# microsoft/foldingdiff

Measured on AMD Instinct MI355X. Metric: backbones/sec (L=128, T=1000, bs=512), higher is better.
Workload: dtype f32 (fp16 hi/lo split operands, 3x v_mfma_f32_{32x32x16,16x16x32}_f16 per product, fp32 accumulate)

## Files before the change

### foldingdiff_amd/csrc/ffn16.hip

```cpp
#include <cstdlib>
#include <type_traits>

#include "fdmi_kernels.h"
#include "img_common.h"
#include "launch_common.h"

namespace fdmi {
namespace ffn {

typedef float f32x4 __attribute__((ext_vector_type(4)));
typedef const __attribute__((address_space(3))) u32x4* lds_cu128_t;
__device__ __forceinline__ unsigned lds_addr(const void* p) { return (unsigned)(unsigned long long)(lds_ptr_t)(const_cast<void*>(p)); }
__device__ __forceinline__ u32x4 lds_u128(unsigned a) { return *(lds_cu128_t)(unsigned long long)a; }
__device__ __forceinline__ f16x8 lds_f16x8(unsigned a) { return __builtin_bit_cast(f16x8, lds_u128(a)); }

__device__ __forceinline__ void swap16(unsigned& vdst, unsigned& src) {
  const auto r = __builtin_amdgcn_permlane16_swap(vdst, src, false, false);
  vdst = r[0];
  src = r[1];
}
__device__ __forceinline__ float quad_sum(float x) {
  unsigned a = __builtin_bit_cast(unsigned, x), b = a;
  swap32(a, b);
  float m = __builtin_bit_cast(float, a) + __builtin_bit_cast(float, b);
  a = __builtin_bit_cast(unsigned, m);
  b = a;
  swap16(a, b);
  return __builtin_bit_cast(float, a) + __builtin_bit_cast(float, b);
}

template <int V> using IC = std::integral_constant<int, V>;
template <int LO, int HI, class F>
__device__ __forceinline__ void static_for(F&& f) {
  if constexpr (LO < HI) {
    f(IC<LO>{});
    static_for<LO + 1, HI>(f);
  }
}

#ifndef FDMI_FFN_DBG
#define FDMI_FFN_DBG 0
#endif
#ifndef FDMI_FFN_ST_AUX
#define FDMI_FFN_ST_AUX 0
#endif
#ifndef FDMI_FFN_PRIO
#define FDMI_FFN_PRIO 2
#endif

__device__ __forceinline__ f32x4 mfma16(const f16x8& a, const f16x8& b, const f32x4& c) {
  return __builtin_amdgcn_mfma_f32_16x16x32_f16(a, b, c, 0, 0, 0);
}

constexpr int NW = 8;
constexpr int TILE = 2048;
constexpr int STEP = 4 * TILE;
constexpr int SPS = 2;
constexpr int STAGE = SPS * STEP;
constexpr int NST = 3;
constexpr int PPW = STAGE / 1024 / NW;
constexpr int OFF_W = 0;
constexpr int OFF_X = NST * STAGE;
__host__ __device__ constexpr int off_p(int nkt) { return OFF_X + NW * nkt * 1024; }

template <int NKT, bool TAIL, bool PROF>
__global__ __launch_bounds__(64 * NW) void ffn16_kernel(FfnArgs p) {
  static_assert(NKT == 12 || NKT == 6, "d_model 384 or 192, intermediate size 2 d_model");
  constexpr int D = 32 * NKT;
  constexpr int NG = NKT;
  constexpr int SPG = 2 * NKT;
  constexpr int STG = SPG / SPS;
  static_assert(STG % NST == 0, "a group is a whole number of ring turns: its first stage always sits in slot 0");
  constexpr int NSA = TAIL ? NKT * NKT / 2 : 0;
  static_assert((NSA / SPS) % NST == 0 && NSA % SPS == 0, "whole ring turns");
  constexpr int W_BYTES = (NSA / SPS + NG * STG) * STAGE;
  constexpr int OFF_P = off_p(NKT);
  constexpr int OFF_P1 = OFF_P + 5 * D * 4;
  extern __shared__ __attribute__((aligned(16))) unsigned char smem[];
  const int tid = threadIdx.x, lane = tid & 63;
  const int wq = __builtin_amdgcn_readfirstlane(tid >> 6);
  const int grp = wq >> 2;
  unsigned smem0 = __builtin_amdgcn_readfirstlane(lds_addr(smem));
  asm volatile("" : "+s"(smem0));
  auto lane_id = [&]() __attribute__((always_inline)) {
    int ln;
    asm volatile("v_mbcnt_lo_u32_b32 %0, -1, 0\n\tv_mbcnt_hi_u32_b32 %0, -1, %0" : "=v"(ln));
    return ln;
  };
  auto lane_off_of = [](int ln) __attribute__((always_inline)) { return (unsigned)((ln >> 4) * 256 + (ln & 15) * 16); };

  {
    float* par = reinterpret_cast<float*>(smem + OFF_P);
    for (int i = tid; i < 2 * D; i += 64 * NW) par[i] = p.bi[i];
    for (int i = tid; i < D; i += 64 * NW) {
      par[2 * D + i] = p.bd[i];
      par[3 * D + i] = p.gamma[i];
      par[4 * D + i] = p.beta[i] * p.out_scale;
      if constexpr (TAIL) {
        par[5 * D + i] = p.bo[i] * (1.0f / p.ao_scale);
        par[6 * D + i] = p.g1[i];
        par[7 * D + i] = p.b1[i] * p.a_scale;
      }
    }
  }

  int w_src = 0, w_slot = 0;
  const __amdgpu_buffer_rsrc_t rs_w = __builtin_amdgcn_make_buffer_rsrc(const_cast<unsigned char*>(p.wimg), 0, W_BYTES, 0x00020000);
  auto issue_w = [&]() __attribute__((always_inline)) {
    const lds_ptr_t dst = (lds_ptr_t)(unsigned long long)(smem0 + OFF_W + (unsigned)__builtin_amdgcn_readfirstlane(w_slot));
    const int so = __builtin_amdgcn_readfirstlane(w_src);
    const int vo = lane_id() * 16;
#pragma unroll
    for (int k = 0; k < PPW; ++k) dma16(rs_w, dst + (wq + NW * k) * 1024, vo, so + (wq + NW * k) * 1024);
    w_src = w_src + STAGE == W_BYTES ? 0 : w_src + STAGE;
    w_slot = w_slot + STAGE == NST * STAGE ? 0 : w_slot + STAGE;
  };

  f16x8 ah[NKT];
  const __amdgpu_buffer_rsrc_t rs_a =
      __builtin_amdgcn_make_buffer_rsrc(const_cast<unsigned char*>(TAIL ? p.cimg : p.aimg), 0, p.a_bytes, 0x00020000);
  const __amdgpu_buffer_rsrc_t rs_h = __builtin_amdgcn_make_buffer_rsrc(const_cast<unsigned char*>(TAIL ? p.hres : p.aimg), 0, p.a_bytes, 0x00020000);
  auto row_off = [&](int r0) __attribute__((always_inline)) {
    const int ln = lane_id();
    const int row = r0 + 16 * wq + (ln & 15);
    return (unsigned)(((row >> 5) * (NKT * 256) + (row & 31)) * 16 + (ln >> 4) * 512);
  };
  u32x4 tl[NKT];
  auto load_hi = [&](int r0) __attribute__((always_inline)) {
    const unsigned hoff = row_off(r0);
#pragma unroll
    for (int kt = 0; kt < NKT; ++kt)
      ah[kt] = __builtin_bit_cast(f16x8, __builtin_amdgcn_raw_buffer_load_b128(rs_a, (int)hoff, kt * 8 * 512, 0));
  };
  auto load_lo = [&](auto KT, unsigned hoff) __attribute__((always_inline)) {
    constexpr int kt = decltype(KT)::value;
    tl[kt] = __builtin_bit_cast(u32x4, __builtin_amdgcn_raw_buffer_load_b128(rs_a, (int)hoff, (kt * 8 + 4) * 512, 0));
  };
  auto commit_lo = [&]() __attribute__((always_inline)) {
    const unsigned ax = smem0 + OFF_X + (unsigned)(wq * NKT * 1024 + lane_id() * 16);
#pragma unroll
    for (int kt = 0; kt < NKT; ++kt) *(__attribute__((address_space(3))) u32x4*)(unsigned long long)(ax + (unsigned)(kt * 1024)) = tl[kt];
  };
  const __amdgpu_buffer_rsrc_t rs_o = __builtin_amdgcn_make_buffer_rsrc(p.out, 0, p.out_bytes, 0x00020000);
  auto load_res = [&](auto KT, unsigned hoff, f32x4 (&Yr)[2 * NKT]) __attribute__((always_inline)) {
    constexpr int kt = decltype(KT)::value;
    Yr[2 * kt] = __builtin_bit_cast(f32x4, __builtin_amdgcn_raw_buffer_load_b128(rs_h, (int)hoff, kt * 8 * 512, 0));
    Yr[2 * kt + 1] = __builtin_bit_cast(f32x4, __builtin_amdgcn_raw_buffer_load_b128(rs_h, (int)hoff, (kt * 8 + 4) * 512, 0));
  };

  const bool rec = PROF && blockIdx.x == 0 && p.stamps != nullptr;
  unsigned long long* stp = PROF ? p.stamps + (size_t)wq * 16 * 16 : nullptr;
  int slot = 0;
#define FD_STAMP(i) do { if (PROF) { if (rec && slot < 16 && lane == 0) stp[slot * 16 + (i)] = __builtin_amdgcn_s_memtime(); } } while (0)
#define FD_SB() __builtin_amdgcn_sched_barrier(0)
#define FD_STAMP_G(i) do { if (PROF) { if (rec && slot == 0 && G == 1 && lane == 0) stp[15 * 16 + (i)] = __builtin_amdgcn_s_memtime(); } } while (0)

  const int n_pass = p.dims ? min(p.panels, __builtin_amdgcn_readfirstlane(p.dims[1]) >> 7) : p.panels;
  if ((int)blockIdx.x >= n_pass) return;
  const float os_up = p.up_scale, os_dn = p.down_scale, hs = 0.5f * p.g_scale;
  const f32x4 zero4 = {0.f, 0.f, 0.f, 0.f};
  f32x4 Y[2 * NKT];
  f32x4 U[4];
  f32x4 Up[4];
  u32x4 uh[2], ul[2];

  load_hi((int)blockIdx.x * 128);
  {
    const unsigned hoff = row_off((int)blockIdx.x * 128);
    static_for<0, NKT>([&](auto KT) __attribute__((always_inline)) { load_lo(KT, hoff); });
    if constexpr (TAIL) static_for<0, NKT>([&](auto KT) __attribute__((always_inline)) { load_res(KT, hoff, Y); });
  }
  issue_w();
  issue_w();
  issue_w();
  FD_WAIT_VM(3 * PPW);
  commit_lo();
  FD_WAIT_VM(2 * PPW);
  barrier_keep_vm();

  auto gelu_piece = [&](auto P, unsigned abq) __attribute__((always_inline)) {
    constexpr int pc = decltype(P)::value, pr = pc >> 2, j = pc & 3;
    const u32x2 b = *(const __attribute__((address_space(3))) u32x2*)(unsigned long long)(abq + (unsigned)((32 * pr + 2 * j) * 4));
    float o0 = __builtin_fmaf(Up[2 * pr + (j >> 1)][2 * (j & 1)], os_up, __builtin_bit_cast(float, (unsigned)b[0]));
    float o1 = __builtin_fmaf(Up[2 * pr + (j >> 1)][2 * (j & 1) + 1], os_up, __builtin_bit_cast(float, (unsigned)b[1]));
#if !(FDMI_FFN_DBG & 1)
    const float h0 = o0 * hs, h1 = o1 * hs;
    o0 = __builtin_fmaf(h0, erf_rational(o0 * 0.70710678118654752440f), h0);
    o1 = __builtin_fmaf(h1, erf_rational(o1 * 0.70710678118654752440f), h1);
#endif
    unsigned a, c;
    split_pair(o0, o1, a, c);
    uh[pr][j] = a;
    ul[pr][j] = c;
  };

  auto steps = [&](auto S0, auto S1, auto GEL, unsigned abq) __attribute__((always_inline)) {
    constexpr int s0 = decltype(S0)::value, s1 = decltype(S1)::value;
    constexpr bool gel = decltype(GEL)::value == 1, pha = decltype(GEL)::value == 2;
    auto stage_top = [&]() __attribute__((always_inline)) {
      FD_WAIT_VM(PPW);
      barrier_keep_vm();
      issue_w();
    };
    f16x8 fx[4], fy[4], xl;
    unsigned a_W, a_X;
    {
      const int ln = lane_id();
      a_W = smem0 + OFF_W + lane_off_of(ln);
      a_X = smem0 + OFF_X + (unsigned)(wq * NKT * 1024 + ln * 16);
      asm volatile("" : "+v"(a_W), "+v"(a_X));
    }
    auto plane_reads = [&](auto S, auto LO, f16x8 (&f)[4]) __attribute__((always_inline)) {
      constexpr int s = decltype(S)::value, lo = decltype(LO)::value;
      constexpr unsigned off = (unsigned)(((s / SPS) % NST) * STAGE + (s % SPS) * STEP + lo * 1024);
#if FDMI_FFN_DBG & 8
      if constexpr (lo == 1) {
#pragma unroll
        for (int t = 0; t < 4; ++t) f[t] = fx[t];
      } else
#endif
#pragma unroll
      for (int t = 0; t < 4; ++t) f[t] = lds_f16x8(a_W + off + (unsigned)(t * TILE));
      if constexpr (pha) {
        if constexpr (lo == 0 && s % (NKT / 2) == 0) xl = lds_f16x8(a_X + (unsigned)((s / (NKT / 2)) * 1024));
      } else {
        if constexpr (lo == 0 && s < NKT) xl = lds_f16x8(a_X + (unsigned)(s * 1024));
      }
    };
    auto mm = [&](auto S, auto WHICH, const f16x8 (&f)[4]) __attribute__((always_inline)) {
      constexpr int s = decltype(S)::value, which = decltype(WHICH)::value;
      if constexpr (pha) {
        constexpr int kt = s / (NKT / 2), q = s % (NKT / 2);
#pragma unroll
        for (int t = 0; t < 4; ++t) Y[4 * q + t] = mfma16(f[t], which == 1 ? xl : ah[kt], Y[4 * q + t]);
      } else if constexpr (s < NKT) {
#if !(FDMI_FFN_DBG & 4)
#pragma unroll
        for (int t = 0; t < 4; ++t) U[t] = mfma16(f[t], which == 1 ? xl : ah[s], U[t]);
#endif
      } else {
#if !(FDMI_FFN_DBG & 2)
        constexpr int pr = (s - NKT) / (NKT / 2), q = (s - NKT) % (NKT / 2);
#pragma unroll
        for (int t = 0; t < 4; ++t) Y[4 * q + t] = mfma16(f[t], __builtin_bit_cast(f16x8, which == 1 ? ul[pr] : uh[pr]), Y[4 * q + t]);
#endif
      }
    };
    plane_reads(S0, IC<0>{}, fx);
    FD_SB();
    static_for<s0, s1>([&](auto S) __attribute__((always_inline)) {
      constexpr int s = decltype(S)::value;
      constexpr bool top = s % SPS == SPS - 1;
      plane_reads(S, IC<1>{}, fy);
      FD_SB();
      if constexpr (top) {
        if (grp == 0) stage_top();
      }
#if FDMI_FFN_PRIO
      __builtin_amdgcn_s_setprio(FDMI_FFN_PRIO);
#endif
      mm(S, IC<0>{}, fx);
      mm(S, IC<1>{}, fx);
#if FDMI_FFN_PRIO
      __builtin_amdgcn_s_setprio(0);
#endif
      FD_SB();
      if constexpr (top) {
        if (grp != 0) stage_top();
      }
      if constexpr (s + 1 < s1) plane_reads(IC<s + 1>{}, IC<0>{}, fx);
      FD_SB();
      if constexpr (gel) {
        if (grp == 0) {
          static_for<0, 8>([&](auto P) __attribute__((always_inline)) {
            if constexpr (1 + decltype(P)::value * (NKT - 2) / 8 == s) gelu_piece(P, abq);
          });
        }
        FD_SB();
      }
      mm(S, IC<2>{}, fy);
      FD_SB();
      if constexpr (gel) {
        if (grp != 0) {
          static_for<0, 8>([&](auto P) __attribute__((always_inline)) {
            if constexpr (1 + decltype(P)::value * (NKT - 2) / 8 == s) gelu_piece(P, abq);
          });
        }
        FD_SB();
      }
    });
  };

  for (int panel = blockIdx.x; panel < n_pass; panel += (int)gridDim.x) {
    FD_STAMP(0);
    if constexpr (TAIL) {
      const int ln = lane_id();
      const int g = ln >> 4;
      const unsigned pb1 = smem0 + OFF_P1 + (unsigned)(8 * g * 4);
      const unsigned ax = smem0 + OFF_X + (unsigned)(wq * NKT * 1024 + ln * 16);
      {
        const float c = p.hres_inv * (1.0f / p.ao_scale);
#pragma unroll
        for (int kt = 0; kt < NKT; ++kt) {
          const u32x4 rh = __builtin_bit_cast(u32x4, Y[2 * kt]), rl = __builtin_bit_cast(u32x4, Y[2 * kt + 1]);
          const u32x4 b0 = lds_u128(pb1 + (unsigned)(kt * 128)), b1 = lds_u128(pb1 + (unsigned)(kt * 128 + 16));
#pragma unroll
          for (int j = 0; j < 2; ++j)
#pragma unroll
            for (int e = 0; e < 4; e += 2) {
              const unsigned hw = rh[2 * j + e / 2], lw = rl[2 * j + e / 2];
              const unsigned bw0 = j == 0 ? b0[e] : b1[e], bw1 = j == 0 ? b0[e + 1] : b1[e + 1];
              float v0 = fma_mix_lo(hw, c, __builtin_bit_cast(float, bw0));
              float v1 = fma_mix_hi(hw, c, __builtin_bit_cast(float, bw1));
              Y[2 * kt + j][e] = fma_mix_lo(lw, c, v0);
              Y[2 * kt + j][e + 1] = fma_mix_hi(lw, c, v1);
            }
        }
      }
      steps(IC<0>{}, IC<NSA>{}, IC<2>{}, 0u);
      const float os_ao = p.ao_scale;
      float sum = 0.f;
#pragma unroll
      for (int t = 0; t < 2 * NKT; ++t)
#pragma unroll
        for (int e = 0; e < 4; ++e) {
          Y[t][e] *= os_ao;
          sum += Y[t][e];
        }
      const float inv_n = 1.0f / (float)D;
      float mean = quad_sum(sum) * inv_n;
      asm volatile("" : "+v"(mean));
      float t2 = 0.f;
#pragma unroll
      for (int t = 0; t < 2 * NKT; ++t)
#pragma unroll
        for (int e = 0; e < 4; ++e) {
          const float dl = Y[t][e] - mean;
          Y[t][e] = dl;
          t2 = __builtin_fmaf(dl, dl, t2);
        }
      const float rstd = (1.0f / sqrtf(__builtin_fmaf(quad_sum(t2), inv_n, p.eps1))) * p.a_scale;
#pragma unroll
      for (int kt = 0; kt < NKT; ++kt) {
        const u32x4 g0 = lds_u128(pb1 + (unsigned)(D * 4 + kt * 128)), g1 = lds_u128(pb1 + (unsigned)(D * 4 + kt * 128 + 16));
        const u32x4 e0 = lds_u128(pb1 + (unsigned)(2 * D * 4 + kt * 128)), e1 = lds_u128(pb1 + (unsigned)(2 * D * 4 + kt * 128 + 16));
        float o[8];
#pragma unroll
        for (int e = 0; e < 4; ++e) {
          o[e] = __builtin_fmaf(Y[2 * kt][e] * rstd, __builtin_bit_cast(float, (unsigned)g0[e]), __builtin_bit_cast(float, (unsigned)e0[e]));
          o[4 + e] = __builtin_fmaf(Y[2 * kt + 1][e] * rstd, __builtin_bit_cast(float, (unsigned)g1[e]), __builtin_bit_cast(float, (unsigned)e1[e]));
        }
        u32x4 hv, lv;
#pragma unroll
        for (int j = 0; j < 4; ++j) {
          unsigned a, b;
          split_pair(o[2 * j], o[2 * j + 1], a, b);
          hv[j] = a;
          lv[j] = b;
        }
        ah[kt] = __builtin_bit_cast(f16x8, hv);
        *(__attribute__((address_space(3))) u32x4*)(unsigned long long)(ax + (unsigned)(kt * 1024)) = lv;
      }
    }
#pragma unroll
    for (int t = 0; t < 2 * NKT; ++t) Y[t] = zero4;
#pragma unroll
    for (int t = 0; t < 4; ++t) U[t] = zero4;
    steps(IC<0>{}, IC<NKT>{}, IC<0>{}, 0u);
    for (int G = 0; G < NG; ++G) {
#pragma unroll
      for (int t = 0; t < 4; ++t) {
        Up[t] = U[t];
        U[t] = zero4;
      }
      unsigned abq = smem0 + OFF_P + (unsigned)((64 * G + 8 * (lane_id() >> 4)) * 4);
      asm volatile("" : "+v"(abq));
      FD_STAMP_G(0);
      FD_STAMP_G(1);
      if (G + 1 < NG) {
#ifdef FDMI_FFN_NOPIPE
        static_for<0, 8>([&](auto P) __attribute__((always_inline)) { gelu_piece(P, abq); });
        steps(IC<0>{}, IC<NKT>{}, IC<0>{}, abq);
#else
        steps(IC<0>{}, IC<NKT>{}, IC<1>{}, abq);
#endif
      } else {
        static_for<0, 8>([&](auto P) __attribute__((always_inline)) { gelu_piece(P, abq); });
      }
      FD_STAMP_G(2);
      steps(IC<NKT>{}, IC<SPG>{}, IC<0>{}, 0u);
      FD_STAMP_G(3);
      if (slot == 0) FD_STAMP(1 + (G < 12 ? G : 11));
    }
    {
      const int ln = lane_id();
      const int g = ln >> 4;
      const unsigned pb = smem0 + OFF_P + (unsigned)((2 * D + 8 * g) * 4);
      const unsigned ax = smem0 + OFF_X + (unsigned)(wq * NKT * 1024 + ln * 16);
      const float ri = p.resid_inv;
      float sum = 0.f;
#pragma unroll
      for (int kt = 0; kt < NKT; ++kt) {
        const u32x4 b0 = lds_u128(pb + (unsigned)(kt * 128)), b1 = lds_u128(pb + (unsigned)(kt * 128 + 16));
        const u32x4 rh = __builtin_bit_cast(u32x4, ah[kt]), rl = lds_u128(ax + (unsigned)(kt * 1024));
#pragma unroll
        for (int j = 0; j < 2; ++j)
#pragma unroll
          for (int e = 0; e < 4; e += 2) {
            const unsigned bw0 = j == 0 ? b0[e] : b1[e], bw1 = j == 0 ? b0[e + 1] : b1[e + 1];
            float v0 = __builtin_fmaf(Y[2 * kt + j][e], os_dn, __builtin_bit_cast(float, bw0));
            float v1 = __builtin_fmaf(Y[2 * kt + j][e + 1], os_dn, __builtin_bit_cast(float, bw1));
            const unsigned hw = rh[2 * j + e / 2], lw = rl[2 * j + e / 2];
            v0 = fma_mix_lo(hw, ri, v0);
            v1 = fma_mix_hi(hw, ri, v1);
            v0 = fma_mix_lo(lw, ri, v0);
            v1 = fma_mix_hi(lw, ri, v1);
            Y[2 * kt + j][e] = v0;
            Y[2 * kt + j][e + 1] = v1;
            sum += v0;
            sum += v1;
          }
      }
      const int next = panel + (int)gridDim.x;
      load_hi(next * 128);
      const unsigned noff = row_off(next * 128);
      const float inv_n = 1.0f / (float)D;
      float mean = quad_sum(sum) * inv_n;
      asm volatile("" : "+v"(mean));
      float t2 = 0.f;
#pragma unroll
      for (int t = 0; t < 2 * NKT; ++t)
#pragma unroll
        for (int e = 0; e < 4; ++e) {
          const float dl = Y[t][e] - mean;
          Y[t][e] = dl;
          t2 = __builtin_fmaf(dl, dl, t2);
        }
      const float rstd = (1.0f / sqrtf(__builtin_fmaf(quad_sum(t2), inv_n, p.eps))) * p.out_scale;
      const unsigned ooff = row_off(panel * 128);
      static_for<0, NKT>([&](auto KT) __attribute__((always_inline)) {
        constexpr int kt = decltype(KT)::value;
        const u32x4 g0 = lds_u128(pb + (unsigned)(D * 4 + kt * 128)), g1 = lds_u128(pb + (unsigned)(D * 4 + kt * 128 + 16));
        const u32x4 e0 = lds_u128(pb + (unsigned)(2 * D * 4 + kt * 128)), e1 = lds_u128(pb + (unsigned)(2 * D * 4 + kt * 128 + 16));
        float o[8];
#pragma unroll
        for (int e = 0; e < 4; ++e) {
          o[e] = __builtin_fmaf(Y[2 * kt][e] * rstd, __builtin_bit_cast(float, (unsigned)g0[e]), __builtin_bit_cast(float, (unsigned)e0[e]));
          o[4 + e] = __builtin_fmaf(Y[2 * kt + 1][e] * rstd, __builtin_bit_cast(float, (unsigned)g1[e]), __builtin_bit_cast(float, (unsigned)e1[e]));
        }
        u32x4 hv, lv;
#pragma unroll
        for (int j = 0; j < 4; ++j) {
          unsigned a, b;
          split_pair(o[2 * j], o[2 * j + 1], a, b);
          hv[j] = a;
          lv[j] = b;
        }
#if FDMI_FFN_DBG & 16
        if (hv[0] == 0x12345678u && lv[1] == 0x9abcdef0u)
#endif
        {
          __builtin_amdgcn_raw_buffer_store_b128(hv, rs_o, (int)ooff, kt * 8 * 512, FDMI_FFN_ST_AUX);
          __builtin_amdgcn_raw_buffer_store_b128(lv, rs_o, (int)ooff, (kt * 8 + 4) * 512, FDMI_FFN_ST_AUX);
        }
        load_lo(KT, noff);
        if constexpr (TAIL) load_res(KT, noff, Y);
        FD_SB();
      });
    }
    FD_STAMP(13);
    FD_WAIT_VM(0);
    commit_lo();
    FD_STAMP(14);
    ++slot;
  }
  FD_WAIT_VM(0);
#undef FD_STAMP
#undef FD_STAMP_G
#undef FD_SB
}

template <int NKT, bool TAIL>
static bool launch(const FfnArgs& p, hipStream_t s) {
  constexpr int SMEM = off_p(NKT) + (TAIL ? 8 : 5) * 32 * NKT * 4;
  static LdsOptIn lds;
  if (!lds({reinterpret_cast<const void*>(&ffn16_kernel<NKT, TAIL, false>), reinterpret_cast<const void*>(&ffn16_kernel<NKT, TAIL, true>)}, SMEM))
    return false;
  int grid = cu_count();
  if (grid > p.panels) grid = p.panels;
  if (grid <= 0) return true;
  if (p.stamps) hipLaunchKernelGGL((ffn16_kernel<NKT, TAIL, true>), dim3(grid), dim3(64 * NW), SMEM, s, p);
  else hipLaunchKernelGGL((ffn16_kernel<NKT, TAIL, false>), dim3(grid), dim3(64 * NW), SMEM, s, p);
  return hipGetLastError() == hipSuccess;
}

}

bool ffn16_supported(int d_model, int d_ff) { return (d_model == 384 || d_model == 192) && d_ff == 2 * d_model; }

bool launch_ffn16(const FfnArgs& p, int d_model, hipStream_t s) {
  if (p.cimg) return d_model == 384 ? ffn::launch<12, true>(p, s) : ffn::launch<6, true>(p, s);
  return d_model == 384 ? ffn::launch<12, false>(p, s) : ffn::launch<6, false>(p, s);
}

}
```

Measured before the change: 81.64.

## Software-pipeline LDS parameter loads and overlap next-panel loads in FFN epilogues

The bias, gamma and beta LDS reads in both layernorm epilogues are double-buffered one k-tile ahead, with scheduling barriers between tiles. The next panel's lo loads now issue during the first residual loop, and its hi loads are split across two points. commit_lo moves ahead of the output store loop, and the output scale multiply is folded into eps. The aim is to hide LDS and global load latency in the epilogue, at the cost of more live registers and extra profiling stamps.

```diff
diff --git a/foldingdiff_amd/csrc/ffn16.hip b/foldingdiff_amd/csrc/ffn16.hip
--- a/foldingdiff_amd/csrc/ffn16.hip
+++ b/foldingdiff_amd/csrc/ffn16.hip
@@ -77,7 +77,7 @@
   constexpr int OFF_P = off_p(NKT);
   constexpr int OFF_P1 = OFF_P + 5 * D * 4;
   extern __shared__ __attribute__((aligned(16))) unsigned char smem[];
-  const int tid = threadIdx.x, lane = tid & 63;
+  const int tid = threadIdx.x;
   const int wq = __builtin_amdgcn_readfirstlane(tid >> 6);
   const int grp = wq >> 2;
   unsigned smem0 = __builtin_amdgcn_readfirstlane(lds_addr(smem));
@@ -126,11 +126,9 @@
     return (unsigned)(((row >> 5) * (NKT * 256) + (row & 31)) * 16 + (ln >> 4) * 512);
   };
   u32x4 tl[NKT];
-  auto load_hi = [&](int r0) __attribute__((always_inline)) {
-    const unsigned hoff = row_off(r0);
-#pragma unroll
-    for (int kt = 0; kt < NKT; ++kt)
-      ah[kt] = __builtin_bit_cast(f16x8, __builtin_amdgcn_raw_buffer_load_b128(rs_a, (int)hoff, kt * 8 * 512, 0));
+  auto load_hi = [&](auto KT, unsigned hoff) __attribute__((always_inline)) {
+    constexpr int kt = decltype(KT)::value;
+    ah[kt] = __builtin_bit_cast(f16x8, __builtin_amdgcn_raw_buffer_load_b128(rs_a, (int)hoff, kt * 8 * 512, 0));
   };
   auto load_lo = [&](auto KT, unsigned hoff) __attribute__((always_inline)) {
     constexpr int kt = decltype(KT)::value;
@@ -151,9 +149,10 @@
   const bool rec = PROF && blockIdx.x == 0 && p.stamps != nullptr;
   unsigned long long* stp = PROF ? p.stamps + (size_t)wq * 16 * 16 : nullptr;
   int slot = 0;
-#define FD_STAMP(i) do { if (PROF) { if (rec && slot < 16 && lane == 0) stp[slot * 16 + (i)] = __builtin_amdgcn_s_memtime(); } } while (0)
+#define FD_STAMP(i) do { if (PROF) { if (rec && slot < 13 && lane_id() == 0) stp[slot * 16 + (i)] = __builtin_amdgcn_s_memtime(); } } while (0)
+#define FD_STAMP_F(i) do { if (PROF) { if (rec && slot < 2 && lane_id() == 0) stp[(14 - slot) * 16 + (i)] = __builtin_amdgcn_s_memtime(); } } while (0)
 #define FD_SB() __builtin_amdgcn_sched_barrier(0)
-#define FD_STAMP_G(i) do { if (PROF) { if (rec && slot == 0 && G == 1 && lane == 0) stp[15 * 16 + (i)] = __builtin_amdgcn_s_memtime(); } } while (0)
+#define FD_STAMP_G(i) do { if (PROF) { if (rec && slot == 0 && G == 1 && lane_id() == 0) stp[15 * 16 + (i)] = __builtin_amdgcn_s_memtime(); } } while (0)
 
   const int n_pass = p.dims ? min(p.panels, __builtin_amdgcn_readfirstlane(p.dims[1]) >> 7) : p.panels;
   if ((int)blockIdx.x >= n_pass) return;
@@ -164,9 +163,9 @@
   f32x4 Up[4];
   u32x4 uh[2], ul[2];
 
-  load_hi((int)blockIdx.x * 128);
   {
     const unsigned hoff = row_off((int)blockIdx.x * 128);
+    static_for<0, NKT>([&](auto KT) __attribute__((always_inline)) { load_hi(KT, hoff); });
     static_for<0, NKT>([&](auto KT) __attribute__((always_inline)) { load_lo(KT, hoff); });
     if constexpr (TAIL) static_for<0, NKT>([&](auto KT) __attribute__((always_inline)) { load_res(KT, hoff, Y); });
   }
@@ -296,37 +295,50 @@
     if constexpr (TAIL) {
       const int ln = lane_id();
       const int g = ln >> 4;
-      const unsigned pb1 = smem0 + OFF_P1 + (unsigned)(8 * g * 4);
-      const unsigned ax = smem0 + OFF_X + (unsigned)(wq * NKT * 1024 + ln * 16);
+      unsigned pb1 = smem0 + OFF_P1 + (unsigned)(8 * g * 4);
+      unsigned ax = smem0 + OFF_X + (unsigned)(wq * NKT * 1024 + ln * 16);
+      asm volatile("" : "+v"(pb1), "+v"(ax));
       {
         const float c = p.hres_inv * (1.0f / p.ao_scale);
-#pragma unroll
-        for (int kt = 0; kt < NKT; ++kt) {
+        u32x4 bq[2][2];
+        auto bias = [&](auto KT) __attribute__((always_inline)) {
+          constexpr int kt = decltype(KT)::value;
+          bq[kt & 1][0] = lds_u128(pb1 + (unsigned)(kt * 128));
+          bq[kt & 1][1] = lds_u128(pb1 + (unsigned)(kt * 128 + 16));
+        };
+        bias(IC<0>{});
+        FD_SB();
+        static_for<0, NKT>([&](auto KT) __attribute__((always_inline)) {
+          constexpr int kt = decltype(KT)::value;
+          if constexpr (kt + 1 < NKT) bias(IC<kt + 1>{});
+          FD_SB();
           const u32x4 rh = __builtin_bit_cast(u32x4, Y[2 * kt]), rl = __builtin_bit_cast(u32x4, Y[2 * kt + 1]);
-          const u32x4 b0 = lds_u128(pb1 + (unsigned)(kt * 128)), b1 = lds_u128(pb1 + (unsigned)(kt * 128 + 16));
 #pragma unroll
           for (int j = 0; j < 2; ++j)
 #pragma unroll
             for (int e = 0; e < 4; e += 2) {
               const unsigned hw = rh[2 * j + e / 2], lw = rl[2 * j + e / 2];
-              const unsigned bw0 = j == 0 ? b0[e] : b1[e], bw1 = j == 0 ? b0[e + 1] : b1[e + 1];
+              const unsigned bw0 = bq[kt & 1][j][e], bw1 = bq[kt & 1][j][e + 1];
               float v0 = fma_mix_lo(hw, c, __builtin_bit_cast(float, bw0));
               float v1 = fma_mix_hi(hw, c, __builtin_bit_cast(float, bw1));
               Y[2 * kt + j][e] = fma_mix_lo(lw, c, v0);
               Y[2 * kt + j][e + 1] = fma_mix_hi(lw, c, v1);
             }
-        }
-      }
+          FD_SB();
+        });
+      }
+      FD_STAMP_F(0);
       steps(IC<0>{}, IC<NSA>{}, IC<2>{}, 0u);
-      const float os_ao = p.ao_scale;
+      FD_STAMP_F(1);
+      float os_ao = p.ao_scale;
+      asm volatile("" : "+s"(os_ao));
+      const float ios = 1.0f / os_ao;
+      const float eps1s = p.eps1 * ios * ios;
       float sum = 0.f;
 #pragma unroll
       for (int t = 0; t < 2 * NKT; ++t)
 #pragma unroll
-        for (int e = 0; e < 4; ++e) {
-          Y[t][e] *= os_ao;
-          sum += Y[t][e];
-        }
+        for (int e = 0; e < 4; ++e) sum += Y[t][e];
       const float inv_n = 1.0f / (float)D;
       float mean = quad_sum(sum) * inv_n;
       asm volatile("" : "+v"(mean));
@@ -339,11 +351,23 @@
           Y[t][e] = dl;
           t2 = __builtin_fmaf(dl, dl, t2);
         }
-      const float rstd = (1.0f / sqrtf(__builtin_fmaf(quad_sum(t2), inv_n, p.eps1))) * p.a_scale;
-#pragma unroll
-      for (int kt = 0; kt < NKT; ++kt) {
-        const u32x4 g0 = lds_u128(pb1 + (unsigned)(D * 4 + kt * 128)), g1 = lds_u128(pb1 + (unsigned)(D * 4 + kt * 128 + 16));
-        const u32x4 e0 = lds_u128(pb1 + (unsigned)(2 * D * 4 + kt * 128)), e1 = lds_u128(pb1 + (unsigned)(2 * D * 4 + kt * 128 + 16));
+      const float rstd = (1.0f / sqrtf(__builtin_fmaf(quad_sum(t2), inv_n, eps1s))) * p.a_scale;
+      FD_STAMP_F(2);
+      u32x4 gq[2][4];
+      auto gamma_beta = [&](auto KT) __attribute__((always_inline)) {
+        constexpr int kt = decltype(KT)::value;
+        gq[kt & 1][0] = lds_u128(pb1 + (unsigned)(D * 4 + kt * 128));
+        gq[kt & 1][1] = lds_u128(pb1 + (unsigned)(D * 4 + kt * 128 + 16));
+        gq[kt & 1][2] = lds_u128(pb1 + (unsigned)(2 * D * 4 + kt * 128));
+        gq[kt & 1][3] = lds_u128(pb1 + (unsigned)(2 * D * 4 + kt * 128 + 16));
+      };
+      gamma_beta(IC<0>{});
+      FD_SB();
+      static_for<0, NKT>([&](auto KT) __attribute__((always_inline)) {
+        constexpr int kt = decltype(KT)::value;
+        if constexpr (kt + 1 < NKT) gamma_beta(IC<kt + 1>{});
+        FD_SB();
+        const u32x4 g0 = gq[kt & 1][0], g1 = gq[kt & 1][1], e0 = gq[kt & 1][2], e1 = gq[kt & 1][3];
         float o[8];
 #pragma unroll
         for (int e = 0; e < 4; ++e) {
@@ -360,13 +384,16 @@
         }
         ah[kt] = __builtin_bit_cast(f16x8, hv);
         *(__attribute__((address_space(3))) u32x4*)(unsigned long long)(ax + (unsigned)(kt * 1024)) = lv;
-      }
+        FD_SB();
+      });
+      FD_STAMP_F(3);
     }
 #pragma unroll
     for (int t = 0; t < 2 * NKT; ++t) Y[t] = zero4;
 #pragma unroll
     for (int t = 0; t < 4; ++t) U[t] = zero4;
     steps(IC<0>{}, IC<NKT>{}, IC<0>{}, 0u);
+    FD_STAMP_F(4);
     for (int G = 0; G < NG; ++G) {
 #pragma unroll
       for (int t = 0; t < 4; ++t) {
@@ -395,19 +422,32 @@
     {
       const int ln = lane_id();
       const int g = ln >> 4;
-      const unsigned pb = smem0 + OFF_P + (unsigned)((2 * D + 8 * g) * 4);
-      const unsigned ax = smem0 + OFF_X + (unsigned)(wq * NKT * 1024 + ln * 16);
+      unsigned pb = smem0 + OFF_P + (unsigned)((2 * D + 8 * g) * 4);
+      unsigned ax = smem0 + OFF_X + (unsigned)(wq * NKT * 1024 + ln * 16);
+      asm volatile("" : "+v"(pb), "+v"(ax));
       const float ri = p.resid_inv;
+      const int next = panel + (int)gridDim.x;
+      const unsigned noff = row_off(next * 128);
+      u32x4 bq[2][3];
+      auto bias_lo = [&](auto KT) __attribute__((always_inline)) {
+        constexpr int kt = decltype(KT)::value;
+        bq[kt & 1][0] = lds_u128(pb + (unsigned)(kt * 128));
+        bq[kt & 1][1] = lds_u128(pb + (unsigned)(kt * 128 + 16));
+        bq[kt & 1][2] = lds_u128(ax + (unsigned)(kt * 1024));
+      };
+      bias_lo(IC<0>{});
+      FD_SB();
       float sum = 0.f;
-#pragma unroll
-      for (int kt = 0; kt < NKT; ++kt) {
-        const u32x4 b0 = lds_u128(pb + (unsigned)(kt * 128)), b1 = lds_u128(pb + (unsigned)(kt * 128 + 16));
-        const u32x4 rh = __builtin_bit_cast(u32x4, ah[kt]), rl = lds_u128(ax + (unsigned)(kt * 1024));
+      static_for<0, NKT>([&](auto KT) __attribute__((always_inline)) {
+        constexpr int kt = decltype(KT)::value;
+        if constexpr (kt + 1 < NKT) bias_lo(IC<kt + 1>{});
+        FD_SB();
+        const u32x4 rh = __builtin_bit_cast(u32x4, ah[kt]), rl = bq[kt & 1][2];
 #pragma unroll
         for (int j = 0; j < 2; ++j)
 #pragma unroll
           for (int e = 0; e < 4; e += 2) {
-            const unsigned bw0 = j == 0 ? b0[e] : b1[e], bw1 = j == 0 ? b0[e + 1] : b1[e + 1];
+            const unsigned bw0 = bq[kt & 1][j][e], bw1 = bq[kt & 1][j][e + 1];
             float v0 = __builtin_fmaf(Y[2 * kt + j][e], os_dn, __builtin_bit_cast(float, bw0));
             float v1 = __builtin_fmaf(Y[2 * kt + j][e + 1], os_dn, __builtin_bit_cast(float, bw1));
             const unsigned hw = rh[2 * j + e / 2], lw = rl[2 * j + e / 2];
@@ -420,10 +460,11 @@
             sum += v0;
             sum += v1;
           }
-      }
-      const int next = panel + (int)gridDim.x;
-      load_hi(next * 128);
-      const unsigned noff = row_off(next * 128);
+        load_lo(KT, noff);
+        FD_SB();
+      });
+      static_for<0, NKT / 2>([&](auto KT) __attribute__((always_inline)) { load_hi(KT, noff); });
+      FD_SB();
       const float inv_n = 1.0f / (float)D;
       float mean = quad_sum(sum) * inv_n;
       asm volatile("" : "+v"(mean));
@@ -437,11 +478,27 @@
           t2 = __builtin_fmaf(dl, dl, t2);
         }
       const float rstd = (1.0f / sqrtf(__builtin_fmaf(quad_sum(t2), inv_n, p.eps))) * p.out_scale;
+      FD_STAMP_F(5);
+      u32x4 gq[2][4];
+      auto gamma_beta = [&](auto KT) __attribute__((always_inline)) {
+        constexpr int kt = decltype(KT)::value;
+        gq[kt & 1][0] = lds_u128(pb + (unsigned)(D * 4 + kt * 128));
+        gq[kt & 1][1] = lds_u128(pb + (unsigned)(D * 4 + kt * 128 + 16));
+        gq[kt & 1][2] = lds_u128(pb + (unsigned)(2 * D * 4 + kt * 128));
+        gq[kt & 1][3] = lds_u128(pb + (unsigned)(2 * D * 4 + kt * 128 + 16));
+      };
+      gamma_beta(IC<0>{});
+      FD_WAIT_VM(NKT / 2);
+      commit_lo();
+      static_for<NKT / 2, NKT>([&](auto KT) __attribute__((always_inline)) { load_hi(KT, noff); });
+      FD_STAMP_F(6);
+      FD_SB();
       const unsigned ooff = row_off(panel * 128);
       static_for<0, NKT>([&](auto KT) __attribute__((always_inline)) {
         constexpr int kt = decltype(KT)::value;
-        const u32x4 g0 = lds_u128(pb + (unsigned)(D * 4 + kt * 128)), g1 = lds_u128(pb + (unsigned)(D * 4 + kt * 128 + 16));
-        const u32x4 e0 = lds_u128(pb + (unsigned)(2 * D * 4 + kt * 128)), e1 = lds_u128(pb + (unsigned)(2 * D * 4 + kt * 128 + 16));
+        if constexpr (kt + 1 < NKT) gamma_beta(IC<kt + 1>{});
+        FD_SB();
+        const u32x4 g0 = gq[kt & 1][0], g1 = gq[kt & 1][1], e0 = gq[kt & 1][2], e1 = gq[kt & 1][3];
         float o[8];
 #pragma unroll
         for (int e = 0; e < 4; ++e) {
@@ -463,20 +520,20 @@
           __builtin_amdgcn_raw_buffer_store_b128(hv, rs_o, (int)ooff, kt * 8 * 512, FDMI_FFN_ST_AUX);
           __builtin_amdgcn_raw_buffer_store_b128(lv, rs_o, (int)ooff, (kt * 8 + 4) * 512, FDMI_FFN_ST_AUX);
         }
-        load_lo(KT, noff);
         if constexpr (TAIL) load_res(KT, noff, Y);
         FD_SB();
       });
     }
     FD_STAMP(13);
     FD_WAIT_VM(0);
-    commit_lo();
+    FD_STAMP_F(7);
     FD_STAMP(14);
     ++slot;
   }
   FD_WAIT_VM(0);
 #undef FD_STAMP
 #undef FD_STAMP_G
+#undef FD_STAMP_F
 #undef FD_SB
 }
 
```

Measured after the change: 81.80 (median of 6 runs). No clear change (+0.2%).
